# ttwang0303/Adaptive-RGBD-Localization-Mappig

Measured on AMD Instinct MI355X. Metric: frames/sec (extract+match+RANSAC-PnP) @640x480, 2000 kp, higher is better.
Workload: dtype u8/i32 (extract, match), f32+f64 (ransac, pnp)

## Files before the change

### adaptive-rgbd-localization-mappig_amd/__init__.py

```python
from __future__ import annotations

import ctypes as C

import numpy as np

from . import _abi
from ._abi import (DETECTOR_ADAPTIVE_FAST, DETECTOR_ADAPTIVE_ORB, DETECTOR_ORB_SLAM2, KNN_FORM_FP4, KNN_FORM_VALU,
                   PYRAMID_FORM_AUTO, PYRAMID_FORM_CHAIN, PYRAMID_FORM_FUSED, PYRAMID_FORM_FUSED_NOBLUR,
                   AdaptiveParams, Calib, Config, DMatch, PnPRansacResult,
                   DMATCH_DTYPE, KP_DTYPE, LANDMARK_DTYPE, LOCAL_MAP_DTYPE, LM_BAD, LM_HAS_OBS, LM_SEEN, LocalMapResult,
                   OrbParams, PAIR_DTYPE, PairResult, RansacParams, Rng, check, load, ptr,
                   ODOMETRY_ADAPTIVE_RBA, ODOMETRY_ADAPTIVE_RICP, ODOMETRY_RANSAC, RicpParams, RicpResult,
                   BA_EDGE_DTYPE, BA_NOTHING, BA_RAN, BaParams, BaResult,
                   FUSE_BAD, FUSE_BEHIND, FUSE_CAND_DTYPE, FUSE_CANDS, FUSE_KF_DTYPE, FUSE_NULL, FUSE_OUTSIDE,
                   CLOUD_DTYPE, CLOUD_INFO_DTYPE, CLOUD_OK, CLOUD_UNFILTERED, ERR_CAPACITY, SOR_INFO_DTYPE,
                   SOR_OK, SOR_SKIPPED, SOR_MAX_K)

__all__ = ["Odometry", "HostFrames", "PinnedResults", "default_config", "load", "KP_DTYPE", "DMATCH_DTYPE", "PAIR_DTYPE", "rng_stream",
           "kabsch", "Calib", "OrbParams", "RansacParams", "Config", "AdaptiveParams", "DETECTOR_ORB_SLAM2",
           "DETECTOR_ADAPTIVE_FAST", "DETECTOR_ADAPTIVE_ORB", "KNN_FORM_FP4", "KNN_FORM_VALU",
           "PYRAMID_FORM_AUTO", "PYRAMID_FORM_FUSED", "PYRAMID_FORM_CHAIN",
           "PYRAMID_FORM_FUSED_NOBLUR", "ODOMETRY_ADAPTIVE_RBA", "ODOMETRY_RANSAC", "ODOMETRY_ADAPTIVE_RICP",
           "RicpParams", "RicpResult", "default_ricp_params", "LANDMARK_DTYPE", "LOCAL_MAP_DTYPE", "LocalMapResult",
           "LM_BAD", "LM_SEEN", "LM_HAS_OBS", "BA_EDGE_DTYPE", "BaParams", "BaResult", "BA_RAN", "BA_NOTHING",
# ... 457 lines not shown
            a.view(np.uint8).fill(fill)
        return out, _abi.PairStageOut(**{k: a.ctypes.data for k, a in out.items()})

    def match_features(self, frames, fill: int = 0x5A):
        kc, n = self.kp_capacity(), len(frames)
        counts = np.array([len(d) for d, _ in frames], np.int32)
        desc = np.full((n, kc, 32), fill, np.uint8)
        xyz = np.full((n, kc, 3), np.nan, np.float32)
        for i, (d, x) in enumerate(frames):
            desc[i, :len(d)] = d
            xyz[i, :len(d)] = x
        out, st = self.match_features_buffers(n, fill)
        check(self.lib.odo_debug_match_features(self.h, n, ptr(counts), ptr(desc), ptr(xyz), C.byref(st)))
        return out

    def pnp_ransac(self, Xw, uv, calib=None, iterations: int = 500, reproj_err: float = 3.0,
                   confidence: float = 0.85):
        Xw = np.ascontiguousarray(Xw, np.float32).reshape(-1, 3)
        uv = np.ascontiguousarray(uv, np.float32).reshape(-1, 2)
        n = Xw.shape[0]
        res = PnPRansacResult()
        mask = np.zeros(max(n, 1), np.uint8)
        good = np.zeros(max(iterations, 1), np.int32)
        cal = calib if calib is not None else self.cfg.calib
        check(self.lib.odo_pnp_ransac(self.h, ptr(Xw), ptr(uv), n, ptr(cal), iterations, reproj_err, confidence,
                                      ptr(res), ptr(mask), ptr(good)))
        return res, mask[:n].astype(bool), good

    def pnp_ransac_batch(self, problems, calib=None, iterations: int = 500, reproj_err: float = 3.0,
                         confidence: float = 0.85):
# ... 180 lines not shown
```

### adaptive-rgbd-localization-mappig_amd/_abi.py

```python
from __future__ import annotations

import ctypes as C
import os

import numpy as np

PKG_DIR = os.path.dirname(os.path.abspath(__file__))
LIB_PATH = os.path.join(PKG_DIR, "libodo_hip.so")

P = C.c_void_p


class OrbKP(C.Structure):
    _fields_ = [("x", C.c_float), ("y", C.c_float), ("size", C.c_float), ("angle", C.c_float),
                ("response", C.c_float), ("octave", C.c_int32), ("class_id", C.c_int32)]


class DMatch(C.Structure):
    _fields_ = [("queryIdx", C.c_int32), ("trainIdx", C.c_int32), ("imgIdx", C.c_int32), ("distance", C.c_float)]


class Calib(C.Structure):
    _fields_ = [(n, C.c_float) for n in ("fx", "fy", "cx", "cy", "k1", "k2", "p1", "p2", "k3",
                                         "depth_factor", "mbf", "th_depth")]
# ... 59 lines not shown
    _fields_ = [("chi2_initial", C.c_double), ("chi2_stage1", C.c_double), ("chi2_final", C.c_double),
                ("iters1", C.c_int32), ("iters2", C.c_int32), ("trials1", C.c_int32), ("trials2", C.c_int32),
                ("n_erase", C.c_int32), ("n_level1", C.c_int32), ("status", C.c_int32), ("pad", C.c_int32)]


class CloudInfo(C.Structure):
    _fields_ = [("status", C.c_int32), ("n_valid", C.c_int32), ("n_points", C.c_int32), ("min_b", C.c_int32 * 3),
                ("div_b", C.c_int32 * 3), ("min_p", C.c_float * 3), ("max_p", C.c_float * 3)]


class PairStageOut(C.Structure):
    _fields_ = [(n, P) for n in ("lm_flags", "qlist", "qcnt", "knn_idx", "knn_dist", "matches", "n_matches",
                                 "good", "n_good", "f2_src", "latch")]


BA_RAN, BA_NOTHING = 0, 1
CLOUD_OK, CLOUD_UNFILTERED = 0, 1
SOR_OK, SOR_SKIPPED = 0, 1
SOR_MAX_K = 64
ODOMETRY_ADAPTIVE_RBA = 0
ODOMETRY_RANSAC = 1
ODOMETRY_ADAPTIVE_RICP = 2
ERR_ARG, ERR_DEVICE, ERR_CAPACITY, ERR_STATE = -1, -2, -3, -4


class KernelForms(C.Structure):
    _fields_ = [("knn", C.c_int32), ("knn_split", C.c_int32), ("ransac_lanes_min_open", C.c_int32),
                ("pyramid", C.c_int32), ("ransac_first_hyps", C.c_int32)]


# ... 83 lines not shown
    "odo_pnp_ransac": (C.c_int, [P, P, P, C.c_int, P, C.c_int, C.c_float, C.c_double, P, P, P]),
    "odo_pnp_ransac_batch": (C.c_int, [P, P, P, P, C.c_int, P, C.c_int, C.c_float, C.c_double, P, P]),
    "odo_gicp_batch": (C.c_int, [P, P, P, P, P, P, C.c_int, C.c_int, C.c_double, P, P, P, P]),
    "odo_gicp": (C.c_int, [P, P, C.c_int, P, C.c_int, P, C.c_int, C.c_double, P, P, P, P]),
    "odo_gicp_covariances": (C.c_int, [P, P, P, C.c_int, P]),
    "odo_gicp_grid_batch": (C.c_int, [P, P, P, P, P, P, C.c_int, C.c_int, C.c_double, C.c_float, P, P, P, P]),
    "odo_gicp_grid_covariances": (C.c_int, [P, P, P, C.c_int, C.c_float, P]),
    "odo_gicp_dense": (C.c_int, [P, P, C.c_int, P, C.c_int, C.c_double, P, P, P, P]),
    "odo_rng_seed": (None, [P, C.c_uint32]),
    "odo_rng_next": (C.c_int32, [P]),
    "odo_debug_pyramid": (C.c_int, [P, C.c_int, P, C.c_size_t]),
    "odo_debug_fast": (C.c_int, [P, C.c_int, C.c_int, P, C.c_int, P]),
    "odo_debug_octree": (C.c_int, [P, C.c_int, C.c_int, P, C.c_int, P]),
    "odo_debug_sort": (C.c_int, [P, P, C.c_int, P]),
    "odo_debug_match_features": (C.c_int, [P, C.c_int, P, P, P, P]),
    "odo_knn_replay_time": (C.c_int, [P, C.c_int, C.POINTER(C.c_float)]),
    "odo_set_timing": (C.c_int, [P, C.c_int]),
    "odo_kernel_timing": (C.c_int, [P, P, P]),
    "odo_step_marks": (C.c_int, [P, C.POINTER(C.c_double), C.c_int]),
    "odo_debug_blur": (C.c_int, [P, C.c_int, P, C.c_size_t]),
    "odo_last_timings": (C.c_int, [P, P, C.c_int, P]),
    "odo_debug_adaptive": (C.c_int, [P, C.c_int, P, P]),
    "odo_set_adaptive_thresholds": (C.c_int, [P, P, C.c_int]),
    "odo_debug_select": (C.c_int, [P, P, C.c_int, C.c_int, C.c_int, P, P]),
    "odo_image_bounds": (C.c_int, [P, P]),
    "odo_chain_poses": (C.c_int, [P, C.c_int, P, P]),
    "odo_write_tum_trajectory": (C.c_int, [C.c_char_p, P, P, C.c_int, C.c_int]),
    "odo_projection_match": (C.c_int, [P, P, P, C.c_int, P, P, P, C.c_int, P, C.c_float, C.c_float, P, P, P]),
    "odo_track_local_map": (C.c_int, [P, P, C.c_int, P, P, C.c_int, C.c_float, C.c_float, P]),
    "odo_get_local_map": (C.c_int, [P, C.c_int, P, P, P, C.c_int]),
# ... 59 lines not shown
```

### adaptive-rgbd-localization-mappig_amd/csrc/k_ransac.hip

```cpp
#include <algorithm>
#include <map>
#include <mutex>
#include <cstdlib>
#include <vector>

#include "odo_device.h"
#include "odo_internal.h"

namespace odo {

struct SortElR {
    uint32_t key;
    uint32_t val;
};

struct GoodPt {
    float sx, sy, sz, tx, ty, tz, w, pad;
};

#define EV_WAVES_C 4
#ifndef EV_H0
#define EV_H0 2
#endif
#define MAX_SAMPLE 8
// ... 32 lines not shown
    RState* st;
    HypRes* hyp;
    int* samples;
    int* ready;
    uint32_t* masks;
    uint32_t* raw;
    int hcap, rawcap;
    uint32_t* best_mask;
    int mask_words;
    odo_pair_result* res;
    float* T12;
    int h_lo, h_hi, no_fold;
    int* open_list;
    int* open_cnt;
    uint32_t* lslab;
};

ODO_INLINE int ld_relaxed(const int* p) { return __hip_atomic_load(p, __ATOMIC_RELAXED, __HIP_MEMORY_SCOPE_AGENT); }
ODO_INLINE void st_relaxed(int* p, int v) { __hip_atomic_store(p, v, __ATOMIC_RELAXED, __HIP_MEMORY_SCOPE_AGENT); }

ODO_INLINE bool set_insert(int (&ids)[MAX_SAMPLE], int& cnt, int id1) {
    bool dup = false;
    int less = 0;
#pragma unroll
    for (int q = 0; q < MAX_SAMPLE; q++) {
        const bool v = q < cnt;
        dup |= v && ids[q] == id1;
        less += (v && ids[q] < id1) ? 1 : 0;
    }
    if (dup) return false;
// ... 574 lines not shown
            for (int u = 0; u < 16; u++) s = (q0 + u < nin) ? s + v[u] : s;
        }
    }
    return s;
}

#define EV_LDS ((size_t)EV_WAVES * 8 * TFC_CAP * sizeof(float))
extern __shared__ __align__(16) uint8_t ev_dyn[];
ODO_INLINE GoodPt load_pt(const GoodPt* P, int k) { return P[k]; }

#ifdef ODO_RANSAC_PROFILE
#define RPROF_MAX 4096
__device__ uint64_t g_rprof[RPROF_MAX * 8];
__device__ uint64_t g_rprof_done;
#endif

ODO_INLINE void try_fold(const RansacBufs& B, const RansacCfg& cfg, int p) {
    RState* S = B.st + p;
    int* ready = B.ready + (size_t)p * B.hcap;
    const HypRes* hyp = B.hyp + (size_t)p * B.hcap;
    const unsigned minInl = (unsigned)cfg.min_inlier_th;
    while (true) {
        if (atomicCAS(&S->lock, 0, 1) != 0) return;
        __threadfence();
        const int H = S->H, ng = S->ng;
        int pos = ld_relaxed(&S->fold_pos), n = ld_relaxed(&S->n), visited = ld_relaxed(&S->visited);
        int valid = ld_relaxed(&S->valid), best = ld_relaxed(&S->best_cnt), best_h = ld_relaxed(&S->best_h);
        float rmse = __int_as_float(ld_relaxed(reinterpret_cast<const int*>(&S->rmse)));
        int sweeps = ld_relaxed(&S->sweeps), fitpts = ld_relaxed(&S->fitpts);
        bool fin = n >= H;
// ... 140 lines not shown
            if (fin) st_relaxed(&S->done, 1);
#ifdef ODO_RANSAC_PROFILE
            if (fin) g_rprof_done = wall_clock64();
#endif
            __threadfence();
            atomicExch(&S->lock, 0);
            __threadfence();
        }
        if (fin) return;
        int rd = 0;
        if (lane == 0) rd = __hip_atomic_load(&ready[pos], __ATOMIC_ACQUIRE, __HIP_MEMORY_SCOPE_AGENT);
        if (!__builtin_amdgcn_readfirstlane(rd)) return;
    }
}

ODO_INLINE void eval_hyps(const RansacBufs& B, const RansacCfg& cfg, int p, int wave, int lane, EvalLds& L,
                          const GoodPt* P, int ng, int words, int H, int hofs, int y0, int hlim, int yrow,
                          int ystride) {
    RState* S = B.st + p;
    const int* smp0 = B.samples + (size_t)p * B.hcap * SREC;
    const TfcSlab TS{reinterpret_cast<float*>(ev_dyn) + (size_t)wave * 8 * TFC_CAP};
    MahalConst K;
    K.raster_cov_x = cfg.raster_cov_x;
    K.raster_cov_y = cfg.raster_cov_y;
    K.depth_cov = *B.latch;
    const float th = cfg.max_mahal * cfg.max_mahal;
    const unsigned minInl = (unsigned)cfg.min_inlier_th;
    const bool efast = __builtin_amdgcn_readfirstlane(S->efast) && ef_fast_cov(K);
    const int hend = min(H, hlim);
    for (int h = hofs + (y0 + yrow) * EV_WAVES + wave; h < hend; h += ystride * EV_WAVES) {
        if (h < B.h_lo || h >= B.h_hi) continue;
        const int* smp = smp0 + (size_t)h * SREC;
        double refinedError = 1e6;
// ... 4 lines not shown
        int nsweep = 0, nfit = 0;
#ifdef ODO_RANSAC_PROFILE
        uint64_t t_tfc = 0, t_get = 0, t_sweep = 0, t0 = 0, t_start = wall_clock64();
        uint64_t tpp[3] = {0, 0, 0};
        int nref = 0, npass = 0;
#define TPP (npass++, tpp)
#define RP_T0() t0 = wall_clock64()
#define RP_ACC(x) x += wall_clock64() - t0
#else
#define RP_T0()
#define RP_ACC(x)
#define TPP nullptr
#endif
        for (int refinements = 1; refinements < 20; refinements++) {
            float tacc = 0.f, tm1 = 0.f, tm2 = 0.f, tc = 0.f;
            RP_T0();
            if (useSample) {
                const int ns = smp[0];
                bool in = false;
                GoodPt g;
                if (lane < ns) {
                    g = load_pt(P, smp[1 + lane]);
                    in = tfc_point_ok(g);
                }
                const uint64_t bal = __ballot(in);
                if (in) stage_pt(TS, lane_rank(bal), g);
                wave_sync();
                nfit += __popcll(bal);
                tfc_fold(TS, __popcll(bal), lane, tacc, tm1, tm2, tc, TPP);
            } else {
// ... 19 lines not shown
                }
                wave_sync();
                tfc_fold(TS, nfill, lane, tacc, tm1, tm2, tc, TPP);
            }
            RP_ACC(t_tfc);
            RP_T0();
            TFC tf;
            tf.accW = __shfl(tacc, 0);
#pragma unroll
            for (int i = 0; i < 3; i++) {
                tf.m1[i] = __shfl(tm1, i);
                tf.m2[i] = __shfl(tm2, 3 * i);
#pragma unroll
                for (int j = 0; j < 3; j++) tf.cov[i][j] = __shfl(tc, 3 * i + j);
            }
            float T[12];
            tf.get(T);
            double Td[12];
#pragma unroll
            for (int i = 0; i < 12; i++) Td[i] = (double)T[i];
            double Zd[6];
            hyp_cov_terms(Td, K, Zd);
            RP_ACC(t_get);
            RP_T0();
            const int dn = ld_relaxed(&S->done);
            double meanError = 0.0;
            unsigned cnt = 0;
            for (int c0 = 0; c0 < ng; c0 += 64) {
                const int k = c0 + lane;
                bool in = false;
                double d = 0.0;
                if (k < ng) {
                    const GoodPt g = load_pt(P, k);
                    if (!(g.sz == 0.0f || g.tx == 0.0f)) {
                        const float x1[3] = {g.sx, g.sy, g.sz}, x2[3] = {g.tx, g.ty, g.tz};
                        d = error_function2_mk(x1, x2, Td, K, Zd, efast);
                        in = !(d > th) && (d >= 0.0);
                    }
                }
                const uint64_t bal = __ballot(in);
                if (in) L.dv[lane_rank(bal)] = d;
                if (lane == 0) {
                    L.nw[c0 >> 5] = (uint32_t)bal;
                    if (c0 + 32 < ng) L.nw[(c0 >> 5) + 1] = (uint32_t)(bal >> 32);
                }
                wave_sync();
                const int nin = __popcll(bal);
                if (lane == 0) meanError = fold_dv(L, nin, meanError);
                cnt += (unsigned)nin;
                wave_sync();
            }
            meanError = __shfl(meanError, 0);
            RP_ACC(t_sweep);
            if (__builtin_amdgcn_readfirstlane(dn)) {
                aborted = true;
                break;
            }
            nsweep++;
#ifdef ODO_RANSAC_PROFILE
            nref++;
#endif
            if (cnt < 3) meanError = 1e9;
            else {
                meanError /= (double)cnt;
                meanError = sqrt(meanError);
            }
            if (cnt < minInl || meanError > (double)cfg.max_mahal) break;
            if (cnt >= refinedCnt && meanError <= refinedError) {
                const unsigned prev = refinedCnt;
#pragma unroll
                for (int i = 0; i < 12; i++) refinedT[i] = T[i];
                refinedError = meanError;
                refinedCnt = cnt;
                for (int w = lane; w < words; w += 64) L.cur[w] = L.nw[w];
                wave_sync();
                useSample = false;
                if (cnt == prev) break;
            } else break;
        }
#ifdef ODO_RANSAC_PROFILE
// ... 48 lines not shown
__global__ void __launch_bounds__(64 * EV_WAVES, EV_MIN_BLOCKS) k_ransac_eval(RansacBufs B, RansacCfg cfg, int hofs, int y0,
                                                                                  int hlim) {
    __builtin_amdgcn_s_setprio(ODO_WAVE_PRIO);
    const int p = blockIdx.x;
    const int wave = threadIdx.x >> 6, lane = threadIdx.x & 63;
    __shared__ EvalLds s_w[EV_WAVES];
    RState* S = B.st + p;
    const int H = S->H;
    if (hofs + (y0 + (int)blockIdx.y) * EV_WAVES >= min(H, hlim)) return;
    __shared__ int s_done;
    if (threadIdx.x == 0) s_done = ld_relaxed(&S->done);
    __syncthreads();
    if (s_done) return;
    const int ng = S->ng, words = S->words;
    const GoodPt* P = B.gpts + (size_t)p * B.match_cap;
    eval_hyps(B, cfg, p, wave, lane, s_w[wave], P, ng, words, H, hofs, y0, hlim, blockIdx.y, gridDim.y);
}

__global__ void __launch_bounds__(256) k_ransac_open(RansacBufs B, int npairs) {
    __shared__ int s_base, s_fast;
    if (threadIdx.x == 0) s_base = 0, s_fast = 1;
    __syncthreads();
    for (int p0 = 0; p0 < npairs; p0 += 256) {
        const int p = p0 + (int)threadIdx.x;
        const bool open = p < npairs && !ld_relaxed(&B.st[p].done);
        if (open && !B.st[p].efast) s_fast = 0;
        const uint64_t bal = __ballot(open);
        __shared__ int s_cnt[4];
        if ((threadIdx.x & 63) == 0) s_cnt[threadIdx.x >> 6] = __popcll(bal);
        __syncthreads();
        int before = 0, tot = 0;
        for (int w = 0; w < 4; w++) {
            if (w < (int)(threadIdx.x >> 6)) before += s_cnt[w];
            tot += s_cnt[w];
        }
        if (open) B.open_list[s_base + before + (int)lane_rank(bal)] = p;
        __syncthreads();
        if (threadIdx.x == 0) s_base += tot;
        __syncthreads();
    }
    if (threadIdx.x == 0) {
        B.open_cnt[0] = s_base;
        B.open_cnt[1] = 0;
        B.open_cnt[2] = s_fast;
    }
}

__global__ void __launch_bounds__(64 * EV_WAVES, EV_MIN_BLOCKS) k_ransac_eval_list(RansacBufs B, RansacCfg cfg, int hofs,
                                                                                   int rows, int max_open) {
    __builtin_amdgcn_s_setprio(ODO_WAVE_PRIO);
    const int wave = threadIdx.x >> 6, lane = threadIdx.x & 63;
    __shared__ EvalLds s_w[EV_WAVES];
    __shared__ int s_item;
    const int cnt = B.open_cnt[0];
    if (cnt > max_open) return;
    const int total = cnt * rows;
    while (true) {
        __syncthreads();
        if (threadIdx.x == 0) s_item = atomicAdd(&B.open_cnt[1], 1);
        __syncthreads();
        const int item = s_item;
        if (item >= total) break;
        const int row = item / cnt, p = B.open_list[item - row * cnt];
        RState* S = B.st + p;
        const int H = S->H;
        if (hofs + row * EV_WAVES >= H || ld_relaxed(&S->done)) continue;
        const GoodPt* P = B.gpts + (size_t)p * B.match_cap;
        eval_hyps(B, cfg, p, wave, lane, s_w[wave], P, S->ng, S->words, H, hofs, row, hofs + (row + 1) * EV_WAVES, 0, 1);
    }
}

ODO_INLINE double readlane_d(double v, int l) {
    const uint64_t u = (uint64_t)__double_as_longlong(v);
    const uint32_t lo = (uint32_t)__builtin_amdgcn_readlane((int)(uint32_t)u, l);
    const uint32_t hi = (uint32_t)__builtin_amdgcn_readlane((int)(uint32_t)(u >> 32), l);
    return __longlong_as_double((long long)(((uint64_t)hi << 32) | lo));
}
#define LN_WAVES 4
#define LN_RS 33
#define LN_TW 18
#ifndef LN_SLOTS
#define LN_SLOTS 32
#endif
// ... 591 lines not shown
    Pack pk;
    auto take = [&](size_t b) {
        const size_t o = pk.add(b);
        return scratch ? (char*)scratch + o : nullptr;
    };
    RansacBufs B{};
    B.gpts = (GoodPt*)take(np * match_cap * sizeof(GoodPt));
    B.st = (RState*)take(np * sizeof(RState));
    B.hyp = (HypRes*)take(np * hc * sizeof(HypRes));
    B.samples = (int*)take(np * hc * SREC * sizeof(int));
    B.ready = (int*)take(np * hc * sizeof(int));
    B.masks = (uint32_t*)take(np * hc * mask_words * 4);
    B.raw = (uint32_t*)take(np * ransac_rawcap(cfg) * 4);
    B.open_list = (int*)take((np + 4) * 4);
    if (scratch) B.open_cnt = B.open_list + npairs;
    B.lslab = (uint32_t*)take(npairs > 1 ? (size_t)ln_groups() * LN_WAVES * 2 * mask_words * 64 * 4 : 0);
    B.hcap = ransac_hcap(cfg);
    B.rawcap = ransac_rawcap(cfg);
    B.match_cap = match_cap;
    B.mask_words = mask_words;
    if (bytes) *bytes = pk.off;
    return B;
}

size_t ransac_scratch_bytes(int npairs, int match_cap, int mask_words, const RansacCfg& cfg) {
    size_t bytes;
    carve(nullptr, npairs, match_cap, mask_words, cfg, &bytes);
    return bytes;
}

typedef std::vector<uint32_t> Mat31;
// ... 204 lines not shown
                       const double* latch, odo_rng* rng_io, uint32_t* best_mask, odo_pair_result* res, float* T12,
                       const odo_ransac_fold_result* d_fold, int h0, int h1, int rank0, const odo_dmatch* good, int ng,
                       int* payload, int words) {
    RansacBufs B = carve(scratch, 1, match_cap, mask_words, cfg);
    B.latch = latch;
    B.rng_io = rng_io;
    B.best_mask = best_mask;
    B.res = res;
    B.T12 = T12;
    hipLaunchKernelGGL(k_hyp_install_dev, dim3(1), dim3(1), 0, st, B, d_fold);
    hipLaunchKernelGGL(k_ransac_final, dim3(1), dim3(64), 0, st, B, cfg);
    hipLaunchKernelGGL(k_hyp_payload, dim3(1), dim3(256), 0, st, B, d_fold, h0, h1, rank0, good, ng, payload, words);
}
int hyp_payload_words(int ng) { return HYP_PAYLOAD_HDR + 4 * std::max(ng, 0); }

}
#ifdef ODO_LANES_PROFILE
extern "C" int odo_lanes_prof_read(uint64_t* out, int n) {
    n = std::min(n, LPROF_MAX);
    if (hipDeviceSynchronize() != hipSuccess) return -1;
    if (hipMemcpyFromSymbol(out, HIP_SYMBOL(odo::g_lprof), (size_t)n * 10 * sizeof(uint64_t)) != hipSuccess) return -1;
    return n;
}
#endif
#ifdef ODO_RANSAC_PROFILE
extern "C" int odo_ransac_prof_read(uint64_t* out, int n, uint64_t* done_t) {
    n = std::min(n, RPROF_MAX);
    if (hipDeviceSynchronize() != hipSuccess) return -1;
    if (hipMemcpyFromSymbol(out, HIP_SYMBOL(odo::g_rprof), (size_t)n * 8 * sizeof(uint64_t)) != hipSuccess) return -1;
    if (hipMemcpyFromSymbol(done_t, HIP_SYMBOL(odo::g_rprof_done), sizeof(uint64_t)) != hipSuccess) return -1;
    std::vector<uint64_t> z((size_t)n * 8, 0);
    (void)hipMemcpyToSymbol(HIP_SYMBOL(odo::g_rprof), z.data(), z.size() * sizeof(uint64_t));
    return n;
}
#endif
```

### adaptive-rgbd-localization-mappig_amd/csrc/odo_hyps.cpp

```cpp
#include "odo_ctx.h"

namespace {

struct PairRansacInput {
    std::vector<odo_dmatch> good;
    int ng = 0, words = 0, kc = 1, n1 = 0, n2 = 0;
    RansacCfg cfg{};
};

int prepare_pair_ransac(const odo_dmatch* m12, int n12, const float* xyz1, int n1, const float* xyz2, int n2,
                        const odo_ransac_params* p, double* latch, PairRansacInput& in, int match_cap) {
    if (n12 < p->min_inlier_th) return 0;
    in.good.clear();
    in.good.reserve(n12);
    for (int i = 0; i < n12; i++) {
        const odo_dmatch& m = m12[i];
        if (m.queryIdx < 0 || m.queryIdx >= n1 || m.trainIdx < 0 || m.trainIdx >= n2)
            return fail(ODO_ERR_ARG, "match index out of range");
        const float zs = xyz1[3 * m.queryIdx + 2], zt = xyz2[3 * m.trainIdx + 2];
        if (p->check_depth) {
            if (std::isnan(zs) || std::isnan(zt)) continue;
            if (zs <= 0 || zt <= 0) continue;
        }
        in.good.push_back(m);
// ... 164 lines not shown
                  s.dev<double>(o.latch), dint + 2, 0, s.dev<odo_rng>(o.rng), dgp.p, s.dev<uint32_t>(o_bm), in.words,
                  s.dev<odo_pair_result>(o_res), dT.as<float>(), 1);
    HIPCHK(hipGetLastError());
    HIPCHK(s.download(st));
    HIPCHK(hipStreamSynchronize(st));
    odo_pair_result r;
    memcpy(&r, s.host<uint8_t>(o_res), sizeof(r));
    memcpy(rng, s.host<uint8_t>(o.rng), sizeof(odo_rng));
    memcpy(T12, r.T12, sizeof(r.T12));
    *rmse = r.rmse;
    *n_inliers = gather_inliers(s.host<uint32_t>(o_bm), in.good, inliers);
    *ok = r.ransac_ok;
    return ODO_OK;
}

int odo_ransac_hyps(odo_ctx* c, const odo_dmatch* m12, int n12, const float* xyz1, int n1, const float* xyz2, int n2,
                    const odo_ransac_params* p, const odo_rng* rng, double* latch, int h0, int h1,
                    odo_hyp_summary* out, int* n_good) {
    if (!c || !p || !rng || !latch || !n_good || n12 < 0 || (n12 && !m12) || h0 < 0 || h1 < h0 ||
        h1 > std::max(p->iterations, 0) || (h1 > h0 && !out))
        return fail(ODO_ERR_ARG, "bad ransac_hyps args");
    for (int h = 0; h < h1 - h0; h++) out[h] = odo_hyp_summary{1e6, 0, 0, {1, 0, 0, 0, 0, 1, 0, 0, 0, 0, 1, 0}};
    int active = 0;
    const int e = hyps_launch(c, m12, n12, xyz1, n1, xyz2, n2, p, rng, latch, h0, h1, n_good, &active);
    if (e || !active) return e;
    HypSession& S = *c->hs;
    PairRansacInput& in = S.in;
    hipStream_t st = c->stream;
    if (h1 > h0) {
        std::vector<double> err(h1 - h0);
// ... 142 lines not shown
```

### adaptive-rgbd-localization-mappig_amd/csrc/odo_internal.h

```cpp
#pragma once

#include <hip/hip_runtime.h>
#include <stddef.h>
#include <stdint.h>
#include <stdlib.h>

#include "../../include/odo_types.h"

namespace odo {

static inline const char* odo_knob(const char* name) {
#ifdef ODO_TUNING
    return getenv(name);
#else
    (void)name;
    return nullptr;
#endif
}

struct Pack {
    size_t off = 0;
    size_t add(size_t bytes) {
        const size_t o = off;
        off = (off + bytes + 255) & ~(size_t)255;
// ... 224 lines not shown
size_t ransac_scratch_bytes(int npairs, int match_cap, int mask_words, const RansacCfg& cfg);
void ransac_read_hyps(hipStream_t st, void* scratch, int match_cap, int mask_words, RansacCfg cfg, int h0, int h1,
                      double* err, int* cnt, float* T);
void launch_ransac_finish(hipStream_t st, void* scratch, int match_cap, int mask_words, RansacCfg cfg,
                          const double* latch, odo_rng* rng_io, uint32_t* best_mask, odo_pair_result* res, float* T12,
                          int best_h, int visited, int valid, int best_cnt, float rmse);
void ransac_export_hyps(hipStream_t st, void* scratch, int match_cap, int mask_words, RansacCfg cfg, int h0, int h1,
                        void* d_block);
void launch_hyp_fold(hipStream_t st, const void* d_all, int H, int iterations, int ng, int min_inl, int sample_size,
                     odo_ransac_fold_result* d_out);
void launch_hyp_finish(hipStream_t st, void* scratch, int match_cap, int mask_words, RansacCfg cfg,
                       const double* latch, odo_rng* rng_io, uint32_t* best_mask, odo_pair_result* res, float* T12,
                       const odo_ransac_fold_result* d_fold, int h0, int h1, int rank0, const odo_dmatch* good, int ng,
                       int* payload, int words);
int hyp_payload_words(int ng);
size_t pnp_edge_bytes();
void launch_pnp(hipStream_t st, const int32_t* f2_src, const float* xyz, const float* kun, const float* ur,
                const int* nkp, int kp_cap, int slot0, FrameCalib cal, const float* T12, const int* pair_valid,
                const int* n_matches, int min_matches, void* edges, odo_pair_result* res, uint8_t* inlier_mask,
                int npairs, const int* sel = nullptr, int sel_val = 0);
void launch_kabsch(hipStream_t st, const float* A, const float* B, int n, float* T);
struct BaArgs {
    int nk, nl, ne, nf;
    const float *Tcw, *Xw, *eobs;
    const int32_t *ekf, *elm, *lstart, *lorder, *kstart, *korder, *pidx;
    const uint8_t* insys;
    float *oT, *oX;
    uint8_t* erase;
    int32_t* counts;
    void* scratch;
// ... 213 lines not shown
```

### include/odo.h

```cpp
#ifndef ODO_H
#define ODO_H

#include <stddef.h>
#include <stdint.h>

#include "odo_types.h"

#ifdef __cplusplus
extern "C" {
#endif

#define ODO_OK 0
#define ODO_ERR_ARG (-1)
#define ODO_ERR_DEVICE (-2)
#define ODO_ERR_CAPACITY (-3)
#define ODO_ERR_STATE (-4)

#define ODO_DETECTOR_ORB_SLAM2 0
#define ODO_DETECTOR_ADAPTIVE_FAST 1
#define ODO_DETECTOR_ADAPTIVE_ORB 2

#define ODO_KNN_FORM_FP4 0
#define ODO_KNN_FORM_VALU 1
#define ODO_PYRAMID_FORM_AUTO 0
// ... 179 lines not shown
int odo_debug_blur(odo_ctx* ctx, int i, uint8_t* out, size_t cap);
int odo_debug_sort(odo_ctx* ctx, const odo_dmatch* in, int n, odo_dmatch* out);

typedef struct odo_pair_stage_out {
    uint8_t* lm_flags;
    int32_t *qlist, *qcnt, *knn_idx, *knn_dist;
    odo_dmatch* matches;
    int32_t* n_matches;
    odo_dmatch* good;
    int32_t *n_good, *f2_src;
    double* latch;
} odo_pair_stage_out;
int odo_debug_match_features(odo_ctx* ctx, int n, const int32_t* counts, const uint8_t* desc, const float* xyz,
                             const odo_pair_stage_out* out);

int odo_knn_replay_time(odo_ctx* ctx, int reps, float* avg_ms);
int odo_debug_adaptive(odo_ctx* ctx, int i, int32_t* t_used, double* thresh);
int odo_set_adaptive_thresholds(odo_ctx* ctx, const double* thresh, int n);
int odo_debug_select(odo_ctx* ctx, const uint32_t* in, int n, int nth, int mode, uint32_t* out, int* n_out);
int odo_set_timing(odo_ctx* ctx, int mode);
int odo_kernel_timing(odo_ctx* ctx, double* avg_ms, long* launches);
int odo_step_marks(odo_ctx* ctx, double* ms, int cap);
int odo_last_timings(odo_ctx* ctx, float* ms, int cap, const char** names);

#ifdef __cplusplus
}
#endif

#endif
```

Measured before the change: 164,900.

## Memoize RANSAC refinement steps by inlier-mask hash across waves

```diff
diff --git a/adaptive-rgbd-localization-mappig_amd/__init__.py b/adaptive-rgbd-localization-mappig_amd/__init__.py
--- a/adaptive-rgbd-localization-mappig_amd/__init__.py
+++ b/adaptive-rgbd-localization-mappig_amd/__init__.py
@@ -495,6 +495,29 @@
         check(self.lib.odo_debug_match_features(self.h, n, ptr(counts), ptr(desc), ptr(xyz), C.byref(st)))
         return out
 
+    def ransac_pairs(self, frames, matches, rp, latch: float, seed: int, pair_base: int = 0):
+        npairs = len(matches)
+        ks = max(max(len(x) for x in frames), 1)
+        ms = max(max(len(m) for m in matches), 1)
+        counts = np.array([len(x) for x in frames], np.int32)
+        xyz = np.full((npairs + 1, ks, 3), np.nan, np.float32)
+        for i, x in enumerate(frames):
+            xyz[i, :len(x)] = x
+        m12 = np.zeros((npairs, ms), DMATCH_DTYPE)
+        n12 = np.array([len(m) for m in matches], np.int32)
+        for i, m in enumerate(matches):
+            m12[i, :len(m)] = m
+        res = np.zeros(npairs, PAIR_DTYPE)
+        masks = np.zeros((npairs, (ms + 31) // 32), np.uint32)
+        inl = np.zeros((npairs, ms), DMATCH_DTYPE)
+        memo = np.zeros(_abi.RANSAC_MEMO_COUNTERS, np.int32)
+        out = _abi.RansacPairsOut(res=res.ctypes.data, masks=masks.ctypes.data, inliers=inl.ctypes.data,
+                                  memo=memo.ctypes.data)
+        check(self.lib.odo_debug_ransac_pairs(self.h, npairs, ptr(m12), ptr(n12), ms, ptr(xyz), ptr(counts), ks,
+                                              C.byref(rp), latch, seed, pair_base, C.byref(out)))
+        inliers = [inl[p, :int(res[p]["n_inliers"])].copy() for p in range(npairs)]
+        return res, inliers, masks, dict(zip(_abi.RANSAC_MEMO_NAMES, (int(v) for v in memo)))
+
     def pnp_ransac(self, Xw, uv, calib=None, iterations: int = 500, reproj_err: float = 3.0,
                    confidence: float = 0.85):
         Xw = np.ascontiguousarray(Xw, np.float32).reshape(-1, 3)
diff --git a/adaptive-rgbd-localization-mappig_amd/_abi.py b/adaptive-rgbd-localization-mappig_amd/_abi.py
--- a/adaptive-rgbd-localization-mappig_amd/_abi.py
+++ b/adaptive-rgbd-localization-mappig_amd/_abi.py
@@ -97,6 +97,12 @@
                                  "good", "n_good", "f2_src", "latch")]
 
 
+class RansacPairsOut(C.Structure):
+    _fields_ = [(n, P) for n in ("res", "masks", "inliers", "memo")]
+
+
+RANSAC_MEMO_COUNTERS = 8
+RANSAC_MEMO_NAMES = ("hits", "waits", "timeouts", "full", "mismatches", "inserts")
 BA_RAN, BA_NOTHING = 0, 1
 CLOUD_OK, CLOUD_UNFILTERED = 0, 1
 SOR_OK, SOR_SKIPPED = 0, 1
@@ -210,6 +216,10 @@
     "odo_debug_octree": (C.c_int, [P, C.c_int, C.c_int, P, C.c_int, P]),
     "odo_debug_sort": (C.c_int, [P, P, C.c_int, P]),
     "odo_debug_match_features": (C.c_int, [P, C.c_int, P, P, P, P]),
+    "odo_debug_ransac_pairs": (C.c_int, [P, C.c_int, P, P, C.c_int, P, P, C.c_int, P, C.c_double, C.c_uint64,
+                                         C.c_uint64, P]),
+    "odo_ransac_memo_hash": (C.c_uint64, [P, C.c_int]),
+    "odo_ransac_memo_slots": (C.c_int, []),
     "odo_knn_replay_time": (C.c_int, [P, C.c_int, C.POINTER(C.c_float)]),
     "odo_set_timing": (C.c_int, [P, C.c_int]),
     "odo_kernel_timing": (C.c_int, [P, P, P]),
diff --git a/adaptive-rgbd-localization-mappig_amd/csrc/k_ransac.hip b/adaptive-rgbd-localization-mappig_amd/csrc/k_ransac.hip
--- a/adaptive-rgbd-localization-mappig_amd/csrc/k_ransac.hip
+++ b/adaptive-rgbd-localization-mappig_amd/csrc/k_ransac.hip
@@ -6,6 +6,7 @@
 
 #include "odo_device.h"
 #include "odo_internal.h"
+#include "../../include/odo.h"
 
 namespace odo {
 
@@ -70,6 +71,8 @@
     int* open_list;
     int* open_cnt;
     uint32_t* lslab;
+    uint32_t* memo;
+    int memo_tabs;
 };
 
 ODO_INLINE int ld_relaxed(const int* p) { return __hip_atomic_load(p, __ATOMIC_RELAXED, __HIP_MEMORY_SCOPE_AGENT); }
@@ -674,6 +677,111 @@
 __device__ uint64_t g_rprof[RPROF_MAX * 8];
 __device__ uint64_t g_rprof_done;
 #endif
+
+#define MEMO_SLOTS 64
+#define MEMO_TABS 31
+#define MEMO_POLLS 128
+#ifndef MEMO_SLEEP0
+#define MEMO_SLEEP0 2
+#endif
+#ifndef MEMO_SLEEP
+#define MEMO_SLEEP 48
+#endif
+#define MEMO_TRIES 4
+#define MEMO_NCTR 8
+#define MEMO_HDR 20
+enum { MEMO_CLAIMED = 1, MEMO_READY = 2, MEMO_DEAD = 3 };
+enum { MC_HIT = 0, MC_WAIT, MC_TIMEOUT, MC_FULL, MC_MISMATCH, MC_INSERT };
+enum { MEMO_COMPUTE = 0, MEMO_OWN, MEMO_TAKE, MEMO_ABORT };
+static_assert(MEMO_SLOTS <= 64 && (MEMO_SLOTS & (MEMO_SLOTS - 1)) == 0, "one lane per slot");
+
+ODO_INLINE __host__ size_t memo_body_words(int mask_words) { return MEMO_HDR + 2 * (size_t)mask_words; }
+ODO_INLINE __host__ size_t memo_tab_words(int mask_words) { return MEMO_SLOTS * (1 + memo_body_words(mask_words)); }
+
+ODO_INLINE __host__ uint32_t memo_fmix(uint32_t x) {
+    x ^= x >> 16;
+    x *= 0x85EBCA6Bu;
+    x ^= x >> 13;
+    x *= 0xC2B2AE35u;
+    x ^= x >> 16;
+    return x;
+}
+ODO_INLINE __host__ void memo_mix(uint32_t word, int i, uint32_t& lo, uint32_t& hi) {
+    const uint32_t k = (uint32_t)(i + 1);
+    lo += memo_fmix(word ^ (k * 0x9E3779B1u));
+    hi += memo_fmix((word + 0x7F4A7C15u) ^ (k * 0x27D4EB2Fu));
+}
+
+ODO_INLINE void memo_count(uint32_t* memo, int which, int lane) {
+    if (lane == 0) atomicAdd(memo + which, 1u);
+}
+ODO_INLINE uint32_t ldu_relaxed(const uint32_t* p) {
+    return __hip_atomic_load(p, __ATOMIC_RELAXED, __HIP_MEMORY_SCOPE_AGENT);
+}
+
+ODO_INLINE int memo_probe(uint32_t* memo, uint32_t* tab, int mw, int words, const uint32_t* cur, uint32_t hlo,
+                          uint32_t hhi, int lane, const int* done, int& slot) {
+    const uint32_t tag = hhi << 2;
+    const int home = (int)(hlo & (MEMO_SLOTS - 1));
+    const int mys = (home + lane) & (MEMO_SLOTS - 1);
+    for (int tries = 0; tries < MEMO_TRIES; tries++) {
+        uint32_t v = 0u;
+        if (lane < MEMO_SLOTS) v = ldu_relaxed(tab + mys);
+        const bool mine = lane < MEMO_SLOTS && (v == 0u || (v & ~3u) == tag);
+        const uint64_t cand = __ballot(mine);
+        if (!cand) {
+            memo_count(memo, MC_FULL, lane);
+            return MEMO_COMPUTE;
+        }
+        const int f = (int)__builtin_ctzll(cand);
+        uint32_t vf = (uint32_t)__builtin_amdgcn_readlane((int)v, f);
+        const int sf = (home + f) & (MEMO_SLOTS - 1);
+        if (f > 0) memo_count(memo, MC_MISMATCH, lane);
+        if (vf == 0u) {
+            uint32_t old = 0u;
+            if (lane == 0) old = atomicCAS(tab + sf, 0u, tag | MEMO_CLAIMED);
+            old = (uint32_t)__builtin_amdgcn_readfirstlane((int)old);
+            if (old == 0u) {
+                memo_count(memo, MC_INSERT, lane);
+                slot = sf;
+                return MEMO_OWN;
+            }
+            if ((old & ~3u) != tag) continue;
+            vf = old;
+        }
+        if ((vf & 3u) == MEMO_CLAIMED) {
+            memo_count(memo, MC_WAIT, lane);
+#pragma unroll
+            for (int i = 0; i < MEMO_SLEEP0; i++) __builtin_amdgcn_s_sleep(127);
+            int polls = 0;
+            while (true) {
+                const uint32_t sv = ldu_relaxed(tab + sf);
+                const int dv = ld_relaxed(done);
+                vf = (uint32_t)__builtin_amdgcn_readfirstlane((int)sv);
+                if ((vf & 3u) != MEMO_CLAIMED) break;
+                if (__builtin_amdgcn_readfirstlane(dv)) return MEMO_ABORT;
+                if (++polls > MEMO_POLLS) {
+                    memo_count(memo, MC_TIMEOUT, lane);
+                    return MEMO_COMPUTE;
+                }
+                __builtin_amdgcn_s_sleep(MEMO_SLEEP);
+            }
+        }
+        if ((vf & 3u) != MEMO_READY) return MEMO_COMPUTE;
+        __builtin_amdgcn_fence(__ATOMIC_ACQUIRE, "agent");
+        const uint32_t* body = tab + MEMO_SLOTS + (size_t)sf * memo_body_words(mw);
+        bool diff = lane == 0 && (ldu_relaxed(body) != hlo || ldu_relaxed(body + 1) != hhi);
+        for (int w = lane; w < words; w += 64) diff |= ldu_relaxed(body + MEMO_HDR + w) != cur[w];
+        if (__ballot(diff)) {
+            memo_count(memo, MC_MISMATCH, lane);
+            return MEMO_COMPUTE;
+        }
+        memo_count(memo, MC_HIT, lane);
+        slot = sf;
+        return MEMO_TAKE;
+    }
+    return MEMO_COMPUTE;
+}
 
 ODO_INLINE void try_fold(const RansacBufs& B, const RansacCfg& cfg, int p) {
     RState* S = B.st + p;
@@ -844,9 +952,10 @@
     }
 }
 
+template <bool MEMO>
 ODO_INLINE void eval_hyps(const RansacBufs& B, const RansacCfg& cfg, int p, int wave, int lane, EvalLds& L,
                           const GoodPt* P, int ng, int words, int H, int hofs, int y0, int hlim, int yrow,
-                          int ystride) {
+                          int ystride, uint32_t* mtab = nullptr) {
     RState* S = B.st + p;
     const int* smp0 = B.samples + (size_t)p * B.hcap * SREC;
     const TfcSlab TS{reinterpret_cast<float*>(ev_dyn) + (size_t)wave * 8 * TFC_CAP};
@@ -881,6 +990,47 @@
 #endif
         for (int refinements = 1; refinements < 20; refinements++) {
             float tacc = 0.f, tm1 = 0.f, tm2 = 0.f, tc = 0.f;
+            float T[12];
+            double meanError = 0.0;
+            unsigned cnt = 0;
+            int mslot = -1;
+            bool taken = false;
+            uint32_t hlo = 0, hhi = 0;
+            const int nfit0 = nfit;
+            if (MEMO && mtab && !useSample) {
+                for (int w = lane; w < words; w += 64) memo_mix(L.cur[w], w, hlo, hhi);
+#pragma unroll
+                for (int o = 32; o > 0; o >>= 1) {
+                    hlo += (uint32_t)__shfl_xor((int)hlo, o);
+                    hhi += (uint32_t)__shfl_xor((int)hhi, o);
+                }
+                hlo = (uint32_t)__builtin_amdgcn_readfirstlane((int)hlo);
+                hhi = (uint32_t)__builtin_amdgcn_readfirstlane((int)hhi);
+                int slot = -1;
+                const int r = memo_probe(B.memo, mtab, B.mask_words, words, L.cur, hlo, hhi, lane, &S->done, slot);
+                if (r == MEMO_ABORT) {
+                    aborted = true;
+                    break;
+                }
+                if (r == MEMO_OWN) mslot = slot;
+                if (r == MEMO_TAKE) {
+                    const uint32_t* body = mtab + MEMO_SLOTS + (size_t)slot * memo_body_words(B.mask_words);
+                    cnt = ldu_relaxed(body + 2);
+                    nfit += (int)ldu_relaxed(body + 3);
+                    meanError = __hiloint2double((int)ldu_relaxed(body + 5), (int)ldu_relaxed(body + 4));
+#pragma unroll
+                    for (int i = 0; i < 12; i++) T[i] = __uint_as_float(ldu_relaxed(body + 6 + i));
+                    for (int w = lane; w < words; w += 64) L.nw[w] = ldu_relaxed(body + MEMO_HDR + B.mask_words + w);
+                    wave_sync();
+                    taken = true;
+                    if (__builtin_amdgcn_readfirstlane(ld_relaxed(&S->done))) {
+                        aborted = true;
+                        break;
+                    }
+                    nsweep++;
+                }
+            }
+            if (!taken) {
             RP_T0();
             if (useSample) {
                 const int ns = smp[0];
@@ -930,7 +1080,6 @@
 #pragma unroll
                 for (int j = 0; j < 3; j++) tf.cov[i][j] = __shfl(tc, 3 * i + j);
             }
-            float T[12];
             tf.get(T);
             double Td[12];
 #pragma unroll
@@ -940,8 +1089,6 @@
             RP_ACC(t_get);
             RP_T0();
             const int dn = ld_relaxed(&S->done);
-            double meanError = 0.0;
-            unsigned cnt = 0;
             for (int c0 = 0; c0 < ng; c0 += 64) {
                 const int k = c0 + lane;
                 bool in = false;
@@ -969,6 +1116,7 @@
             meanError = __shfl(meanError, 0);
             RP_ACC(t_sweep);
             if (__builtin_amdgcn_readfirstlane(dn)) {
+                if (MEMO && mslot >= 0 && lane == 0) st_relaxed(reinterpret_cast<int*>(mtab + mslot), (int)((hhi << 2) | MEMO_DEAD));
                 aborted = true;
                 break;
             }
@@ -980,6 +1128,31 @@
             else {
                 meanError /= (double)cnt;
                 meanError = sqrt(meanError);
+            }
+            if (MEMO && mslot >= 0) {
+                uint32_t* body = mtab + MEMO_SLOTS + (size_t)mslot * memo_body_words(B.mask_words);
+                if (lane == 0) {
+                    body[0] = hlo;
+                    body[1] = hhi;
+                    body[2] = cnt;
+                    body[3] = (uint32_t)(nfit - nfit0);
+                    *reinterpret_cast<double*>(body + 4) = meanError;
+                }
+                if (lane < 12) {
+                    float v = T[0];
+#pragma unroll
+                    for (int i = 1; i < 12; i++)
+                        if (lane == i) v = T[i];
+                    body[6 + lane] = __float_as_uint(v);
+                }
+                for (int w = lane; w < words; w += 64) {
+                    body[MEMO_HDR + w] = L.cur[w];
+                    body[MEMO_HDR + B.mask_words + w] = L.nw[w];
+                }
+                __builtin_amdgcn_fence(__ATOMIC_RELEASE, "agent");
+                __builtin_amdgcn_wave_barrier();
+                if (lane == 0) st_relaxed(reinterpret_cast<int*>(mtab + mslot), (int)((hhi << 2) | MEMO_READY));
+            }
             }
             if (cnt < minInl || meanError > (double)cfg.max_mahal) break;
             if (cnt >= refinedCnt && meanError <= refinedError) {
@@ -1058,7 +1231,7 @@
     if (s_done) return;
     const int ng = S->ng, words = S->words;
     const GoodPt* P = B.gpts + (size_t)p * B.match_cap;
-    eval_hyps(B, cfg, p, wave, lane, s_w[wave], P, ng, words, H, hofs, y0, hlim, blockIdx.y, gridDim.y);
+    eval_hyps<false>(B, cfg, p, wave, lane, s_w[wave], P, ng, words, H, hofs, y0, hlim, blockIdx.y, gridDim.y);
 }
 
 __global__ void __launch_bounds__(256) k_ransac_open(RansacBufs B, int npairs) {
@@ -1083,6 +1256,13 @@
         if (threadIdx.x == 0) s_base += tot;
         __syncthreads();
     }
+    if (B.memo) {
+        const int nt = min(s_base, B.memo_tabs);
+        const size_t tw = memo_tab_words(B.mask_words);
+        if (threadIdx.x < MEMO_NCTR) B.memo[threadIdx.x] = 0;
+        for (int i = threadIdx.x; i < nt * MEMO_SLOTS; i += 256)
+            B.memo[MEMO_NCTR + (size_t)(i / MEMO_SLOTS) * tw + (i % MEMO_SLOTS)] = 0;
+    }
     if (threadIdx.x == 0) {
         B.open_cnt[0] = s_base;
         B.open_cnt[1] = 0;
@@ -1105,12 +1285,14 @@
         __syncthreads();
         const int item = s_item;
         if (item >= total) break;
-        const int row = item / cnt, p = B.open_list[item - row * cnt];
+        const int row = item / cnt, at = item - row * cnt, p = B.open_list[at];
         RState* S = B.st + p;
         const int H = S->H;
         if (hofs + row * EV_WAVES >= H || ld_relaxed(&S->done)) continue;
         const GoodPt* P = B.gpts + (size_t)p * B.match_cap;
-        eval_hyps(B, cfg, p, wave, lane, s_w[wave], P, S->ng, S->words, H, hofs, row, hofs + (row + 1) * EV_WAVES, 0, 1);
+        uint32_t* mtab = at < B.memo_tabs ? B.memo + MEMO_NCTR + (size_t)at * memo_tab_words(B.mask_words) : nullptr;
+        eval_hyps<true>(B, cfg, p, wave, lane, s_w[wave], P, S->ng, S->words, H, hofs, row, hofs + (row + 1) * EV_WAVES, 0, 1,
+                        mtab);
     }
 }
 
@@ -1732,7 +1914,11 @@
     B.raw = (uint32_t*)take(np * ransac_rawcap(cfg) * 4);
     B.open_list = (int*)take((np + 4) * 4);
     if (scratch) B.open_cnt = B.open_list + npairs;
-    B.lslab = (uint32_t*)take(npairs > 1 ? (size_t)ln_groups() * LN_WAVES * 2 * mask_words * 64 * 4 : 0);
+    const size_t lanes_b = (size_t)ln_groups() * LN_WAVES * 2 * mask_words * 64 * 4;
+    B.memo_tabs = npairs > 1 ? std::min(npairs, MEMO_TABS) : 0;
+    const size_t memo_b = B.memo_tabs ? (MEMO_NCTR + B.memo_tabs * memo_tab_words(mask_words)) * 4 : 0;
+    B.lslab = (uint32_t*)take(npairs > 1 ? std::max(lanes_b, memo_b) : 0);
+    B.memo = B.memo_tabs ? B.lslab : nullptr;
     B.hcap = ransac_hcap(cfg);
     B.rawcap = ransac_rawcap(cfg);
     B.match_cap = match_cap;
@@ -1967,6 +2153,14 @@
 }
 int hyp_payload_words(int ng) { return HYP_PAYLOAD_HDR + 4 * std::max(ng, 0); }
 
+void ransac_read_memo(hipStream_t st, void* scratch, int npairs, int match_cap, int mask_words, RansacCfg cfg,
+                      int32_t* out) {
+    static_assert(ODO_RANSAC_MEMO_COUNTERS == MEMO_NCTR, "odo.h's counter block");
+    const RansacBufs B = carve(scratch, npairs, match_cap, mask_words, cfg);
+    for (int i = 0; i < MEMO_NCTR; i++) out[i] = 0;
+    if (B.memo) (void)hipMemcpyAsync(out, B.memo, MEMO_NCTR * sizeof(int32_t), hipMemcpyDeviceToHost, st);
+}
+
 }
 #ifdef ODO_LANES_PROFILE
 extern "C" int odo_lanes_prof_read(uint64_t* out, int n) {
@@ -1976,6 +2170,12 @@
     return n;
 }
 #endif
+extern "C" uint64_t odo_ransac_memo_hash(const uint32_t* mask, int words) {
+    uint32_t lo = 0, hi = 0;
+    for (int i = 0; mask && i < words; i++) odo::memo_mix(mask[i], i, lo, hi);
+    return ((uint64_t)hi << 32) | lo;
+}
+extern "C" int odo_ransac_memo_slots(void) { return MEMO_SLOTS; }
 #ifdef ODO_RANSAC_PROFILE
 extern "C" int odo_ransac_prof_read(uint64_t* out, int n, uint64_t* done_t) {
     n = std::min(n, RPROF_MAX);
diff --git a/adaptive-rgbd-localization-mappig_amd/csrc/odo_hyps.cpp b/adaptive-rgbd-localization-mappig_amd/csrc/odo_hyps.cpp
--- a/adaptive-rgbd-localization-mappig_amd/csrc/odo_hyps.cpp
+++ b/adaptive-rgbd-localization-mappig_amd/csrc/odo_hyps.cpp
@@ -202,6 +202,78 @@
     return ODO_OK;
 }
 
+int odo_debug_ransac_pairs(odo_ctx* c, int npairs, const odo_dmatch* m12, const int32_t* n12, int match_stride,
+                           const float* xyz, const int32_t* counts, int kp_stride, const odo_ransac_params* p,
+                           double latch, uint64_t seed, uint64_t pair_base, const odo_ransac_pairs_out* out) {
+    if (!c || !m12 || !n12 || !xyz || !counts || !p || !out || !out->res || !out->masks || !out->inliers || !out->memo)
+        return fail(ODO_ERR_ARG, "ransac_pairs: null argument");
+    if (npairs < 2 || npairs > 4096 || match_stride < 1 || kp_stride < 1 || std::isnan(latch))
+        return fail(ODO_ERR_ARG, "ransac_pairs: at least 2 pairs, positive strides, a latch value");
+    if (match_stride > 8192) return fail(ODO_ERR_CAPACITY, "ransac_pairs: at most 8192 matches per pair");
+    for (int i = 0; i <= npairs; i++)
+        if (counts[i] < 0 || counts[i] > kp_stride) return fail(ODO_ERR_ARG, "ransac_pairs: frame count outside 0 .. kp_stride");
+    for (int i = 0; i < npairs; i++)
+        if (n12[i] < 0 || n12[i] > match_stride) return fail(ODO_ERR_ARG, "ransac_pairs: match count outside 0 .. match_stride");
+    int e;
+    if ((e = sync_all(c))) return e;
+    const size_t KS = (size_t)kp_stride, MS = (size_t)match_stride;
+    const int words = (match_stride + 31) / 32;
+    std::vector<PairRansacInput> in(npairs);
+    std::vector<int> run(npairs);
+    for (int i = 0; i < npairs; i++) {
+        double lat = latch;
+        run[i] = prepare_pair_ransac(m12 + i * MS, n12[i], xyz + i * KS * 3, counts[i], xyz + (i + 1) * KS * 3,
+                                     counts[i + 1], p, &lat, in[i], c->match_cap);
+        if (run[i] < 0) return run[i];
+    }
+    const RansacCfg cfg = ransac_cfg(*p);
+    hipStream_t st = c->stream;
+    Staged s;
+    const size_t o_xyz = s.add((size_t)(npairs + 1) * KS * 12), o_m = s.add(npairs * MS * sizeof(odo_dmatch)),
+                 o_g = s.add(npairs * MS * 8), o_int = s.add((size_t)3 * npairs * sizeof(int)), o_lat = s.add(sizeof(double));
+    s.mark_inputs_end();
+    s.mark_outputs_begin();
+    const size_t o_res = s.add(npairs * sizeof(odo_pair_result)), o_bm = s.add((size_t)npairs * words * 4);
+    if ((e = s.reserve(c, c->arena))) return e;
+    DevBuf dT(c->arena, (size_t)npairs * 16 * sizeof(float)),
+        scr(c->arena, ransac_scratch_bytes(npairs, match_stride, words, cfg));
+    ARENA_CHECK(c->arena);
+    memset(s.h, 0, s.in_end);
+    memcpy(s.host<float>(o_xyz), xyz, (size_t)(npairs + 1) * KS * 12);
+    int* ints = s.host<int>(o_int);
+    for (int i = 0; i < npairs; i++) {
+        const int ng = run[i] > 0 ? in[i].ng : 0;
+        ints[i] = ints[npairs + i] = ng;
+        ints[2 * npairs + i] = run[i] > 0 ? 1 : 0;
+        uint64_t* gl = s.host<uint64_t>(o_g) + i * MS;
+        for (int k = 0; k < ng; k++) {
+            s.host<odo_dmatch>(o_m)[i * MS + k] = in[i].good[k];
+            uint32_t bits;
+            memcpy(&bits, &in[i].good[k].distance, 4);
+            gl[k] = ((uint64_t)(uint32_t)k << 32) | bits;
+        }
+    }
+    memcpy(s.host<double>(o_lat), &latch, sizeof(double));
+    HIPCHK(s.upload(st));
+    HIPCHK(hipMemsetAsync(s.d + s.out_begin, 0, s.pk.off - s.out_begin, st));
+    int* dint = s.dev<int>(o_int);
+    launch_ransac_raw(st, scr.p, npairs, match_stride, words, cfg, seed, pair_base, nullptr);
+    launch_ransac(st, s.dev<uint8_t>(o_g), dint, dint + npairs, s.dev<odo_dmatch>(o_m), s.dev<float>(o_xyz), kp_stride, 0,
+                  match_stride, cfg, s.dev<double>(o_lat), dint + 2 * npairs, 0, nullptr, scr.p, s.dev<uint32_t>(o_bm),
+                  words, s.dev<odo_pair_result>(o_res), dT.as<float>(), npairs);
+    HIPCHK(hipGetLastError());
+    ransac_read_memo(st, scr.p, npairs, match_stride, words, cfg, out->memo);
+    HIPCHK(s.download(st));
+    HIPCHK(hipStreamSynchronize(st));
+    memcpy(out->res, s.host<uint8_t>(o_res), npairs * sizeof(odo_pair_result));
+    memcpy(out->masks, s.host<uint8_t>(o_bm), (size_t)npairs * words * 4);
+    for (int i = 0; i < npairs; i++) {
+        in[i].good.resize(run[i] > 0 ? in[i].ng : 0);
+        gather_inliers(out->masks + (size_t)i * words, in[i].good, out->inliers + i * MS);
+    }
+    return ODO_OK;
+}
+
 int odo_ransac_hyps(odo_ctx* c, const odo_dmatch* m12, int n12, const float* xyz1, int n1, const float* xyz2, int n2,
                     const odo_ransac_params* p, const odo_rng* rng, double* latch, int h0, int h1,
                     odo_hyp_summary* out, int* n_good) {
diff --git a/adaptive-rgbd-localization-mappig_amd/csrc/odo_internal.h b/adaptive-rgbd-localization-mappig_amd/csrc/odo_internal.h
--- a/adaptive-rgbd-localization-mappig_amd/csrc/odo_internal.h
+++ b/adaptive-rgbd-localization-mappig_amd/csrc/odo_internal.h
@@ -262,6 +262,8 @@
                        const odo_ransac_fold_result* d_fold, int h0, int h1, int rank0, const odo_dmatch* good, int ng,
                        int* payload, int words);
 int hyp_payload_words(int ng);
+void ransac_read_memo(hipStream_t st, void* scratch, int npairs, int match_cap, int mask_words, RansacCfg cfg,
+                      int32_t* out);
 size_t pnp_edge_bytes();
 void launch_pnp(hipStream_t st, const int32_t* f2_src, const float* xyz, const float* kun, const float* ur,
                 const int* nkp, int kp_cap, int slot0, FrameCalib cal, const float* T12, const int* pair_valid,
diff --git a/include/odo.h b/include/odo.h
--- a/include/odo.h
+++ b/include/odo.h
@@ -217,6 +217,19 @@
 int odo_debug_match_features(odo_ctx* ctx, int n, const int32_t* counts, const uint8_t* desc, const float* xyz,
                              const odo_pair_stage_out* out);
 
+#define ODO_RANSAC_MEMO_COUNTERS 8
+typedef struct odo_ransac_pairs_out {
+    odo_pair_result* res;
+    uint32_t* masks;
+    odo_dmatch* inliers;
+    int32_t* memo;
+} odo_ransac_pairs_out;
+int odo_debug_ransac_pairs(odo_ctx* ctx, int npairs, const odo_dmatch* m12, const int32_t* n12, int match_stride,
+                           const float* xyz, const int32_t* counts, int kp_stride, const odo_ransac_params* p,
+                           double latch, uint64_t seed, uint64_t pair_base, const odo_ransac_pairs_out* out);
+uint64_t odo_ransac_memo_hash(const uint32_t* mask, int words);
+int odo_ransac_memo_slots(void);
+
 int odo_knn_replay_time(odo_ctx* ctx, int reps, float* avg_ms);
 int odo_debug_adaptive(odo_ctx* ctx, int i, int32_t* t_used, double* thresh);
 int odo_set_adaptive_thresholds(odo_ctx* ctx, const double* thresh, int n);
```

Measured after the change: 164,000. No clear change (-0.5%).
